# consilience-dev/llm-map-reduce-summarizer

Measured on AMD Instinct MI355X. Metric: chunks/sec (whole node) + end-to-end wall-clock, 10h transcript, Llama-3-8B, higher is better.
Workload: dtype bf16

## Files before the change

### llm_map_reduce_summarizer_amd/csrc/kernels/stream_gemm.hip

```cpp
#include "ar_common.h"

namespace {
enum { EPI_BF16 = 0, EPI_F32_PARTIAL = 1, EPI_SWIGLU = 2, EPI_SWIGLU_SPLIT = 3, EPI_RESID_SPLIT = 4 };
constexpr int SS_PARTS = 8;
constexpr int KBLK = 128;
constexpr int LDS_XTRA = 3 * 1024;
constexpr int LDS_BUDGET = 160 * 1024 - LDS_XTRA;

struct NormArgs {
    const float* ssq;
    int ssq_tiles;
    float inv_k, eps;
    bf16* resid;
    int ldr;
    float* ssp;
    int slab_m;
    mrsum_ar::TPPush tp;
};

template <int N>
__device__ __forceinline__ void wait_vmcnt() {
    static_assert(N >= 0 && N < 64, "vmcnt range");
    __builtin_amdgcn_s_waitcnt((N & 15) | (7 << 4) | (15 << 8) | ((N >> 4) << 14));
}
// ... 692 lines not shown
    f32x4 acc[MT];
#pragma unroll
    for (int m = 0; m < MT; ++m) acc[m] = f32x4{0.f, 0.f, 0.f, 0.f};

#pragma unroll
    for (int s = 0; s < D - 1; ++s) ISSUEP(s, min(s, nkb - 1));

    const uint32_t kb0 = (uint32_t)(ks / KBLK);
    uint32_t ex[P13_EXCAP], exkb = ~0u;
    if constexpr (BITS == 13) {
#pragma unroll
        for (int c = 0; c < P13_EXCAP; ++c) ex[c] = ~0u;
        if (nex > 0) {
#pragma unroll
            for (int c = 0; c < P13_EXCAP; ++c) {
                if (c < nex) ex[c] = __builtin_amdgcn_readfirstlane(exlist[ex0 + c]);
                const uint32_t kbc = ex[c] >> 18;
                if (kbc >= kb0) exkb = min(exkb, kbc);
            }
        }
    }

    const uint32_t base4 = (uint32_t)(base7 - 1) * 0x01010101u;
    const int r = lane & 15, g = lane >> 4;
    for (int j = 0; j < nkb; ++j) {
        if (j + D - 2 < nkb) wait_vmcnt<NI * (D - 2)>();
        else wait_vmcnt<0>();
        raw_barrier();
        if (j + D - 1 < nkb) ISSUEP((j + D - 1) % D, j + D - 1);
        const char* wl = lds + (j % D) * SLOT + w * TILE;
        const char* xl = lds + (j % D) * SLOT + WBYTES;
        const u32x4 lo0 = *reinterpret_cast<const u32x4*>(wl + 16 * lane);
        const u32x4 lo1 = *reinterpret_cast<const u32x4*>(wl + 1024 + 16 * lane);
        const u32x4 nb = *reinterpret_cast<const u32x4*>(wl + F::NIB + 16 * lane);
        u32x4 av[4];
        if constexpr (BITS == 14) {
            const u32x2 s2 = *reinterpret_cast<const u32x2*>(wl + F::TOP + 8 * lane);
            av[0] = p14_frag<0>(lo0[0], lo0[1], nb[0], s2.x, base4);
            av[1] = p14_frag<1>(lo0[2], lo0[3], nb[1], s2.x, base4);
            av[2] = p14_frag<0>(lo1[0], lo1[1], nb[2], s2.y, base4);
            av[3] = p14_frag<1>(lo1[2], lo1[3], nb[3], s2.y, base4);
        } else {
            const uint32_t sg = *reinterpret_cast<const uint32_t*>(wl + F::TOP + 4 * lane);
            av[0] = p13_frag<0>(lo0[0], lo0[1], nb[0], sg, base4);
            av[1] = p13_frag<1>(lo0[2], lo0[3], nb[1], sg, base4);
            av[2] = p13_frag<2>(lo1[0], lo1[1], nb[2], sg, base4);
            av[3] = p13_frag<3>(lo1[2], lo1[3], nb[3], sg, base4);
            if (kb0 + (uint32_t)j == exkb) {
                const uint32_t cur = exkb;
                exkb = ~0u;
#pragma unroll
                for (int c = 0; c < P13_EXCAP; ++c) {
                    uint32_t xc = ex[c];
                    asm volatile("" : "+s"(xc));
                    const uint32_t kbc = xc >> 18;
                    if (kbc == cur) {
                        const int sl = (xc >> 7) & 31;
                        const uint32_t v = lane == (int)((xc >> 12) & 63) ? (xc & 127u) << (8 + 16 * (sl & 1)) : 0u;
#pragma unroll
                        for (int i = 0; i < 4; ++i)
#pragma unroll
                            for (int d = 0; d < 4; ++d) av[i][d] |= sl >> 1 == 4 * i + d ? v : 0u;
                    } else if (kbc > cur) {
                        exkb = min(exkb, kbc);
                    }
                }
            }
        }
#pragma unroll
        for (int i = 0; i < 4; ++i) {
#pragma unroll
            for (int m = 0; m < MT; ++m) {
                const u32x4 bv = *reinterpret_cast<const u32x4*>(xl + img_off(16 * m + r, 4 * i + g));
                acc[m] = __builtin_amdgcn_mfma_f32_16x16x32_bf16(__builtin_bit_cast(bf16x8, av[i]),
                                                                 __builtin_bit_cast(bf16x8, bv), acc[m], 0, 0, 0);
            }
        }
    }
#undef ISSUEP

    stream_epilogue<MT, EPI, WPB>(acc, lds, s_ss, n0, M, out, ldo, parts, counters, e);
}

template <int BITS>
static int launch_packed(const void* x, int ldx, const void* W, int base7, const int* exoff, const uint32_t* exlist,
                         int N, int K, int M, void* out, int ldo, int epi, int splits, int wpb, void* parts,
                         int* counters, const float* ssq, int ssq_tiles, float eps, void* resid, int ldr, float* ssp,
                         void* ar, hipStream_t s) {
    if (M <= 0) return 0;
    if (wpb < 4 || wpb > 8 || M > 64 || K % KBLK || N % (16 * wpb) || splits < 1 || (K / KBLK) % splits ||
        epi < EPI_BF16 || epi > EPI_RESID_SPLIT || base7 < 1 || base7 > 128 - Packed<BITS>::WINDOW || ar)
        return (int)hipErrorInvalidValue;
    if (BITS == 13 && (!exoff || !exlist || K / KBLK >= 0x3fff)) return (int)hipErrorInvalidValue;
    const bool split_epi = epi == EPI_SWIGLU_SPLIT || epi == EPI_RESID_SPLIT;
    if (epi != EPI_F32_PARTIAL && !split_epi && splits != 1) return (int)hipErrorInvalidValue;
    if (split_epi && (!parts || !counters)) return (int)hipErrorInvalidValue;
    if (epi == EPI_RESID_SPLIT && (!resid || !ssp || ldr % 4)) return (int)hipErrorInvalidValue;
    if (ssq && (ssq_tiles <= 0 || ssq_tiles % (4 * SS_PARTS))) return (int)hipErrorInvalidValue;
    NormArgs e;
    e.ssq = ssq; e.ssq_tiles = ssq_tiles; e.inv_k = 1.f / (float)K; e.eps = eps;
    e.resid = (bf16*)resid; e.ldr = ldr; e.ssp = ssp; e.slab_m = 0;
    e.tp = mrsum_ar::tp_push_of(nullptr);
    const int kper = K / splits;
    const int mt = (M + 15) / 16;
    dim3 grid(N / (16 * wpb), splits), block(64 * wpb);
    auto X = (const bf16*)x;
    auto Wp = (const unsigned char*)W;
    auto P = (float*)parts;
#define L14(MT_, EPI_, WPB_)                                                                                      \
    stream_packed_kernel<BITS, MT_, EPI_, WPB_><<<grid, block, 0, s>>>(X, ldx, Wp, base7, exoff, exlist, K, M, out, \
                                                                       ldo, kper, P, counters, e)
#define BY_WPB14(MT_, EPI_)                         \
    switch (wpb) {                                  \
        case 4: L14(MT_, EPI_, 4); break;           \
        case 5: L14(MT_, EPI_, 5); break;           \
        case 6: L14(MT_, EPI_, 6); break;           \
        case 7: L14(MT_, EPI_, 7); break;           \
        default: L14(MT_, EPI_, 8); break;          \
    }
#define BY_EPI14(MT_)                                                      \
    if (epi == EPI_BF16) { BY_WPB14(MT_, EPI_BF16) }                       \
    else if (epi == EPI_F32_PARTIAL) { BY_WPB14(MT_, EPI_F32_PARTIAL) }    \
    else if (epi == EPI_SWIGLU) { BY_WPB14(MT_, EPI_SWIGLU) }              \
    else if (epi == EPI_SWIGLU_SPLIT) { BY_WPB14(MT_, EPI_SWIGLU_SPLIT) }  \
    else { BY_WPB14(MT_, EPI_RESID_SPLIT) }
    switch (mt) {
        case 1: BY_EPI14(1); break;
        case 2: BY_EPI14(2); break;
        case 3: BY_EPI14(3); break;
        default: BY_EPI14(4); break;
    }
#undef BY_EPI14
#undef BY_WPB14
#undef L14
    return (int)hipGetLastError();
}

MRSUM_API int mrsum_stream_p14(const void* x, int ldx, const void* W, int base7, int N, int K, int M, void* out,
                               int ldo, int epi, int splits, int wpb, void* parts, int* counters, const float* ssq,
                               int ssq_tiles, float eps, void* resid, int ldr, float* ssp, void* ar, hipStream_t s) {
    return launch_packed<14>(x, ldx, W, base7, nullptr, nullptr, N, K, M, out, ldo, epi, splits, wpb, parts, counters,
                             ssq, ssq_tiles, eps, resid, ldr, ssp, ar, s);
}

MRSUM_API int mrsum_stream_p13(const void* x, int ldx, const void* W, int base7, const int* exoff,
                               const unsigned int* exlist, int N, int K, int M, void* out, int ldo, int epi, int splits,
                               int wpb, void* parts, int* counters, const float* ssq, int ssq_tiles, float eps,
                               void* resid, int ldr, float* ssp, void* ar, hipStream_t s) {
    return launch_packed<13>(x, ldx, W, base7, exoff, exlist, N, K, M, out, ldo, epi, splits, wpb, parts, counters,
                             ssq, ssq_tiles, eps, resid, ldr, ssp, ar, s);
}

namespace {
__global__ __launch_bounds__(256) void p14_max_kernel(const uint4* __restrict__ W, size_t n16, int* __restrict__ stats) {
    uint32_t m = 0;
    for (size_t i = (size_t)blockIdx.x * blockDim.x + threadIdx.x; i < n16; i += (size_t)gridDim.x * blockDim.x) {
        const uint4 v = W[i];
        const uint32_t d[4] = {v.x, v.y, v.z, v.w};
#pragma unroll
        for (int c = 0; c < 4; ++c) m = max(m, max((d[c] >> 8) & 0x7fu, (d[c] >> 24) & 0x7fu));
    }
#pragma unroll
    for (int o = 32; o > 0; o >>= 1) m = max(m, (uint32_t)__shfl_xor((int)m, o, 64));
    if ((threadIdx.x & 63) == 0) atomicMax(stats, (int)m);
}

__global__ __launch_bounds__(64) void p14_pack_kernel(const bf16* __restrict__ W, int K, unsigned char* __restrict__ P,
                                                      int* __restrict__ stats) {
    const int lane = threadIdx.x, r = lane & 15, g = lane >> 4;
    const int nkb = K / KBLK;
    const size_t tile = blockIdx.x;
    const int G = (int)(tile / nkb), kb = (int)(tile % nkb);
    const int base7 = max(stats[0] - 30, 1);
    const uint4* src = reinterpret_cast<const uint4*>(W + (size_t)(16 * G + r) * K + (size_t)kb * KBLK + 8 * g);
    uint32_t lo[8], nb[4], s2[2] = {0u, 0u};
    int bad = 0;
#pragma unroll
    for (int i = 0; i < 4; ++i) {
        const uint4 v = src[4 * i];
        const uint32_t d[4] = {v.x, v.y, v.z, v.w};
        lo[2 * i] = lo[2 * i + 1] = nb[i] = 0u;
#pragma unroll
        for (int el = 0; el < 8; ++el) {
            const uint32_t wv = (d[el >> 1] >> (16 * (el & 1))) & 0xffffu;
            const int e7 = (wv >> 8) & 0x7f, c = e7 ? e7 - base7 + 1 : 0;
            bad += e7 && (c < 1 || c > 31);
            const uint32_t c5 = (uint32_t)c & 31u, sg = wv >> 15;
            const int b = el & 3, q = 2 * (i & 1) + (el >> 2);
            lo[2 * i + (el >> 2)] |= (wv & 0xffu) << (8 * b);
            nb[i] |= (c5 & 15u) << (8 * b + 4 * (el >> 2));
            s2[i >> 1] |= (c5 >> 4) << (8 * b + 4 - q) | sg << (8 * b + 7 - (q == 3 ? 7 : q));
        }
    }
    unsigned char* t = P + tile * P14_TILE;
    *reinterpret_cast<uint4*>(t + 16 * lane) = make_uint4(lo[0], lo[1], lo[2], lo[3]);
    *reinterpret_cast<uint4*>(t + 1024 + 16 * lane) = make_uint4(lo[4], lo[5], lo[6], lo[7]);
    *reinterpret_cast<uint4*>(t + P14_NIB + 16 * lane) = make_uint4(nb[0], nb[1], nb[2], nb[3]);
    *reinterpret_cast<uint2*>(t + P14_TWO + 8 * lane) = make_uint2(s2[0], s2[1]);
    if (bad) atomicAdd(stats + 1, bad);
}
}

MRSUM_API int mrsum_p14_pack(const void* W, int N, int K, void* packed, int* stats, hipStream_t s) {
    if (N <= 0 || K <= 0 || N % 16 || K % KBLK || !W || !packed || !stats) return (int)hipErrorInvalidValue;
    hipError_t rc = hipMemsetAsync(stats, 0, 2 * sizeof(int), s);
    if (rc != hipSuccess) return (int)rc;
    const size_t n16 = (size_t)N * K / 8;
    const int blocks = (int)((n16 + 255) / 256 < 4096 ? (n16 + 255) / 256 : 4096);
    p14_max_kernel<<<blocks, 256, 0, s>>>((const uint4*)W, n16, stats);
    p14_pack_kernel<<<(unsigned)((size_t)(N / 16) * (K / KBLK)), 64, 0, s>>>((const bf16*)W, K, (unsigned char*)packed,
                                                                              stats);
    return (int)hipGetLastError();
}

namespace {
__global__ __launch_bounds__(64) void p13_pack_kernel(const bf16* __restrict__ W, int K, unsigned char* __restrict__ P,
                                                      int* __restrict__ stats, int* __restrict__ excnt,
                                                      uint32_t* __restrict__ exbuf) {
    const int lane = threadIdx.x, r = lane & 15, g = lane >> 4;
    const int nkb = K / KBLK;
    const size_t tile = blockIdx.x;
    const int G = (int)(tile / nkb), kb = (int)(tile % nkb);
    const int base7 = max(stats[0] - 14, 1);
    const uint4* src = reinterpret_cast<const uint4*>(W + (size_t)(16 * G + r) * K + (size_t)kb * KBLK + 8 * g);
    uint32_t lo[8], nb[4], sg = 0u;
    int nexc = 0;
#pragma unroll
    for (int i = 0; i < 4; ++i) {
        const uint4 v = src[4 * i];
        const uint32_t d[4] = {v.x, v.y, v.z, v.w};
        lo[2 * i] = lo[2 * i + 1] = nb[i] = 0u;
#pragma unroll
        for (int el = 0; el < 8; ++el) {
// ... 41 lines not shown
```

### llm_map_reduce_summarizer_amd/ops/hip.py

```python

from __future__ import annotations

import ctypes
import os
from typing import Optional

import torch

from ._lib import kernels_lib
from .reference import Fp8Weight

_c_int, _c_float, _vp = ctypes.c_int, ctypes.c_float, ctypes.c_void_p

_SIGS = {
    "mrsum_rmsnorm": [_vp, _vp, _vp, _c_int, _c_int, _c_int, _c_int, _c_float, _vp],
    "mrsum_add_rmsnorm": [_vp, _vp, _vp, _vp, _c_int, _c_int, _c_int, _c_int, _c_float, _vp],
    "mrsum_rmsnorm_fp8": [_vp, _vp, _vp, _vp, _vp, _c_int, _c_int, _c_int, _c_int, _c_float, _c_int, _vp],
    "mrsum_rope_kv": [_vp, _c_int, _c_int, _vp, _vp, _vp, _c_int, _vp, _vp, _vp, _c_int, _c_int, _c_int, _c_int,
                      _c_int, _c_int, _vp],
    "mrsum_rope_kv_parts": [_vp, _c_int, _vp, _c_int, _c_int, _vp, _vp, _vp, _c_int, _vp, _vp, _vp, _c_int,
                            _c_int, _c_int, _c_int, _c_int, _vp],
    "mrsum_swiglu": [_vp, _vp, _c_int, _c_int, _vp],
    "mrsum_kv_scatter": [_vp, _c_int, _c_int, _c_int, _vp, _vp, _vp, _vp, _c_int, _vp],
    "mrsum_embed": [_vp, _vp, _vp, _c_int, _c_int, _c_int, _vp],
    "mrsum_attn_prefill": [_vp, _c_int, _vp, _vp, _c_int, _c_int, _vp, _c_int, _c_int, _c_int, _c_int, _c_float, _vp],
    "mrsum_attn_prefill_paged": [_vp, _c_int, _vp, _vp, _c_int, _c_int, _vp, _c_int, _c_int, _c_int, _c_int, _c_float,
                                 _vp,
                                 _vp, _vp, _c_int, _vp, _vp, _c_int, _vp],
    "mrsum_attn_decode_mfma": [_vp, _c_int, _vp, _vp, _vp, _c_int, _vp, _vp, _vp, _vp, _c_int, _c_int, _c_int,
                               _c_int, _c_int, _c_int, _c_int, _c_float, _vp, _c_int, _vp],
    "mrsum_attn_decode_rope": [_vp, _c_int, _vp, _vp, _vp, _vp, _c_int, _vp, _vp, _vp, _vp, _c_int, _c_int,
                               _c_int, _c_int, _c_int, _c_int, _c_int, _c_float, _vp, _c_int, _vp],
    "mrsum_skinny_gemm": [_vp, _c_int, _vp, _c_int, _c_int, _c_int, _vp, _c_int, _c_int, _c_int, _c_int, _vp, _c_int,
                          _c_float, _vp, _c_int, _vp, _vp, _c_int, _vp],
    "mrsum_skinny_resid_capacity_w": [_c_int],
    "mrsum_skinny_lds": [_vp, _c_int, _vp, _c_int, _c_int, _c_int, _vp, _c_int, _c_int, _c_int, _c_int, _vp],
    "mrsum_stream_gemm": [_vp, _c_int, _vp, _c_int, _c_int, _c_int, _vp, _c_int, _c_int, _c_int, _c_int, _vp, _vp,
                          _vp, _c_int, _c_float, _vp, _c_int, _vp, _c_int, _vp, _vp],
    "mrsum_stream_fp8": [_vp, _c_int, _vp, _vp, _c_int, _c_int, _c_int, _vp, _c_int, _c_int, _c_int, _c_int, _vp, _vp,
                         _vp, _c_int, _c_float, _vp, _c_int, _vp, _vp, _vp],
    "mrsum_stream_p14": [_vp, _c_int, _vp, _c_int, _c_int, _c_int, _c_int, _vp, _c_int, _c_int, _c_int, _c_int, _vp,
                         _vp, _vp, _c_int, _c_float, _vp, _c_int, _vp, _vp, _vp],
    "mrsum_p14_pack": [_vp, _c_int, _c_int, _vp, _vp, _vp],
    "mrsum_stream_p13": [_vp, _c_int, _vp, _c_int, _vp, _vp, _c_int, _c_int, _c_int, _vp, _c_int, _c_int, _c_int,
                         _c_int, _vp, _vp, _vp, _c_int, _c_float, _vp, _c_int, _vp, _vp, _vp],
    "mrsum_p13_pack": [_vp, _c_int, _c_int, _vp, _vp, _vp, _vp, _vp],
    "mrsum_skinny_fp8": [_vp, _c_int, _vp, _vp, _c_int, _c_int, _c_int, _vp, _c_int, _c_int, _c_int, _c_int, _vp,
                         _c_int, _c_float, _vp, _c_int, _vp, _vp, _c_int, _vp],
    "mrsum_skinny_fp8_resid_capacity": [],
    "mrsum_quant_fp8_rows": [_vp, _c_int, _vp, _vp, _c_int, _c_int, _vp],
    "mrsum_add_rmsnorm_parts": [_vp, _c_int, _vp, _vp, _vp, _c_int, _c_int, _c_int, _c_float, _vp],
    "mrsum_sample_keys": [_vp, _c_int, _c_int, _c_int, _c_int, _vp, _vp, _vp, _vp, _vp],
    "mrsum_sample_finish": [_vp, _vp, _vp, _vp, _vp, _vp, _c_int, _vp, _vp, _c_int, _vp],
    "mrsum_gemm": [_vp, _c_int, _vp, _c_int, _vp, _c_int, _c_int, _c_int, _c_int, _c_int, _c_int, _vp, _vp, _c_int,
                   _c_int, _vp],
    "mrsum_sample": [_vp, _c_int, _c_int, _c_int, _vp, _vp, _vp, _vp, _vp, _vp, _vp, _vp, _vp, _c_int, _vp, _vp,
                     _vp],
    "mrsum_penalize": [_vp, _c_int, _c_int, _c_int, _c_int, _vp, _c_int, _vp, _vp, _vp, _vp, _vp, _vp],
    "mrsum_penalize_scan": [_vp, _c_int, _c_int, _c_int, _c_int, _vp, _c_int, _vp, _vp, _vp, _vp, _vp, _vp],
    "mrsum_constrain": [_vp, _c_int, _c_int, _c_int, _c_int, _vp, _vp, _c_int, _vp, _vp, _vp, _vp, _vp, _vp, _vp],
    "mrsum_sample_finish_stops": [_vp, _vp, _vp, _vp, _vp, _vp, _c_int, _vp, _vp, _vp, _c_int, _vp],
    "mrsum_sample_keys_filtered": [_vp, _c_int, _c_int, _c_int, _vp, _vp, _vp, _vp, _vp, _vp, _vp, _vp, _vp, _vp],
    "mrsum_logprobs": [_vp, _c_int, _c_int, _c_int, _vp, _vp, _vp, _c_int, _vp, _vp, _vp, _vp, _vp, _vp, _vp, _vp],
    "mrsum_logprobs_pick": [_vp, _c_int, _c_int, _c_int, _vp, _c_int, _vp, _vp, _vp, _vp, _c_int, _vp],
    "mrsum_sample_thresh": [_vp, _c_int, _c_int, _c_int, _vp, _vp, _vp, _vp, _vp, _vp, _vp],
    "mrsum_sample_filtered": [_vp, _c_int, _c_int, _c_int, _vp, _vp, _vp, _vp, _vp, _vp, _vp, _vp, _vp, _vp, _vp,
                              _vp, _vp, _c_int, _vp, _vp, _vp],
}

_fns = {}


def _fn(name: str):
    f = _fns.get(name)
    if f is None:
        lib = kernels_lib()
        f = getattr(lib, name)
        f.argtypes = _SIGS[name]
        f.restype = ctypes.c_int
        _fns[name] = f
    return f


def _stream() -> int:
    return torch.cuda.current_stream().cuda_stream


def _p(t: Optional[torch.Tensor]) -> Optional[int]:
    return None if t is None else t.data_ptr()


DEBUG_SYNC = os.environ.get("MRSUM_DEBUG_SYNC", "0") == "1"


def _check(rc: int, name: str) -> None:
    if rc != 0:
        raise RuntimeError("%s launch failed: hipError %d" % (name, rc))
    if DEBUG_SYNC and not torch.cuda.is_current_stream_capturing():
        try:
            torch.cuda.synchronize()
        except RuntimeError as e:
            raise RuntimeError("%s: device error after the launch: %s" % (name, e)) from e


def _req(cond: bool, msg: str) -> None:
    if not cond:
        raise ValueError(msg)


def _bf16_cuda(*ts: torch.Tensor) -> None:
    for t in ts:
        _req(t.is_cuda and t.dtype == torch.bfloat16, "expected a bf16 CUDA tensor, got %s %s" % (t.dtype, t.device))


def _i32(*ts: torch.Tensor) -> None:
    for t in ts:
        _req(t.is_cuda and t.dtype == torch.int32 and t.is_contiguous(), "expected a contiguous int32 CUDA tensor")


def _rows_ok(x: torch.Tensor) -> None:
    _req(x.dim() == 2 and x.stride(1) == 1 and x.stride(0) % 8 == 0 and x.data_ptr() % 16 == 0,
         "expected a 2-D row-major tensor with 16-byte aligned rows")


def rmsnorm(x: torch.Tensor, w: torch.Tensor, eps: float, out: Optional[torch.Tensor] = None) -> torch.Tensor:
    _bf16_cuda(x, w)
    _rows_ok(x)
    T, D = x.shape
    _req(w.numel() == D and w.is_contiguous() and D % 8 == 0 and D <= 16384, "rmsnorm: bad weight / D")
    if out is None:
# ... 706 lines not shown
    return out


def _norm_args(x, norm):
    if norm is None:
        return None, 0, 0.0
    ssq, eps = norm
    _req(ssq.is_cuda and ssq.dtype == torch.float32 and ssq.is_contiguous() and ssq.dim() == 2
         and ssq.shape[0] == x.shape[0] and ssq.shape[1] % 32 == 0, "deferred norm: ssq must be fp32 [M, 32k]")
    return _p(ssq), ssq.shape[1], float(eps)


def _resid_args(x, N, epi, resid, ssp):
    if epi != EPI_RESID_SPLIT:
        return None, 0, None
    M = x.shape[0]
    _bf16_cuda(resid)
    _rows_ok(resid)
    _req(resid.shape == (M, N) and ssp is not None and ssp.dtype == torch.float32 and ssp.is_contiguous()
         and ssp.dim() == 2 and ssp.shape[0] == M, "resid split: residual [M, N] bf16 and ssp fp32 [M, tiles]")
    return _p(resid), resid.stride(0), _p(ssp)


def _stream_gemm(x, w, out, epi, splits, ldo, wpb, parts=None, counters=None, norm=None, resid=None, ssp=None,
                 ar=None):
    _bf16_cuda(x, w)
    _rows_ok(x)
    M, K = x.shape
    N = w.shape[0]
    if M > SKINNY_MAX_M and epi in (EPI_BF16, EPI_F32_PARTIAL, EPI_SWIGLU) and norm is None:
        ch = STREAM_TALL_M
        for r0 in range(0, M, ch):
            r1 = min(M, r0 + ch)
            if r1 - r0 > SKINNY_MAX_M:
                tw = tall_wpb(N, r1 - r0, splits)
                if tw is not None:
                    o = out[:, r0:r1] if epi == EPI_F32_PARTIAL else out[r0:r1]
                    _stream_launch(x[r0:r1], w, o, epi, splits, ldo, tw, None, None, None, None, None,
                                   M if epi == EPI_F32_PARTIAL else 0)
                    continue
            for c0 in range(r0, r1, SKINNY_MAX_M):
                c1 = min(r1, c0 + SKINNY_MAX_M)
                o = out[:, c0:c1] if epi == EPI_F32_PARTIAL else out[c0:c1]
                _stream_launch(x[c0:c1], w, o, epi, splits, ldo, wpb, None, None, None, None, None,
                               M if epi == EPI_F32_PARTIAL else 0)
        return out
    return _stream_launch(x, w, out, epi, splits, ldo, wpb, parts, counters, norm, resid, ssp, 0, ar)


STREAM_TALL_M = 128
_TALL_WPB = {6: (4, 5, 6), 8: (4, 5)}


def tall_wpb(N: int, M: int, splits: int) -> Optional[int]:
    mt = 6 if M <= 96 else 8
    best, key = None, None
    for wpb in _TALL_WPB[mt]:
        if N % (16 * wpb):
            continue
        grid = N // (16 * wpb) * splits
        k = (round(grid / (-(-grid // N_CU) * N_CU), 3), wpb)
        if key is None or k > key:
            best, key = wpb, k
    return best


def _stream_launch(x, w, out, epi, splits, ldo, wpb, parts, counters, norm, resid, ssp, slab_m, ar=None):
    M, K = x.shape
    N = w.shape[0]
    _req(w.is_contiguous() and w.shape[1] == K, "stream_gemm: weight must be [N, K] contiguous")
    tall_ok = M <= 128 and epi in (EPI_BF16, EPI_F32_PARTIAL, EPI_SWIGLU) and norm is None
    _req(1 <= M and (M <= SKINNY_MAX_M or tall_ok) and K % 128 == 0 and 4 <= wpb <= 8 and N % (16 * wpb) == 0
         and (K // 128) % splits == 0, "stream_gemm: unsupported shape M=%d N=%d K=%d S=%d wpb=%d"
         % (M, N, K, splits, wpb))
    if epi in (EPI_SWIGLU_SPLIT, EPI_RESID_SPLIT):
        _req(parts is not None and parts.shape == (splits, M, N) and parts.dtype == torch.float32
             and counters is not None and counters.numel() >= N // (16 * wpb), "stream_gemm: split-K scratch")
    if epi == EPI_RESID_SPLIT:
        _req(ssp.shape[1] == N // (16 * wpb), "stream_gemm: ssp tiles")
    sq, tiles, eps = _norm_args(x, norm)
    rp, ldr, sp = _resid_args(x, N, epi, resid, ssp)
    packed_ok = M <= SKINNY_MAX_M and not slab_m and ar is None
    p3 = p13_lookup(w) if _P13 else None
    if p3 is not None and packed_ok and p13_takes(p3.role, M):
        STATS["stream_p14"] += 1
        STATS["stream_p13"] += 1
        _check(_fn("mrsum_stream_p13")(_p(x), x.stride(0), _p(p3.packed), p3.base7, _p(p3.exoff), _p(p3.exlist), N, K,
                                       M, _p(out), ldo, epi, splits, wpb, _p(parts), _p(counters), sq, tiles, eps, rp,
                                       ldr, sp, None, _stream()), "stream_p13")
        return out
    pw = p14_lookup(w) if _P14 else None
    if pw is not None and packed_ok and p14_takes(pw.role, M):
        STATS["stream_p14"] += 1
        _check(_fn("mrsum_stream_p14")(_p(x), x.stride(0), _p(pw.packed), pw.base7, N, K, M, _p(out), ldo, epi, splits,
                                       wpb, _p(parts), _p(counters), sq, tiles, eps, rp, ldr, sp, None, _stream()),
               "stream_p14")
        return out
    STATS["stream_bf16"] += 1
    _check(_fn("mrsum_stream_gemm")(_p(x), x.stride(0), _p(w), N, K, M, _p(out), ldo, epi, splits, wpb, _p(parts),
                                    _p(counters), sq, tiles, eps, rp, ldr, sp, slab_m, ar, _stream()), "stream_gemm")
    return out


P14_ROLES = ("qkv", "o", "gate_up", "down", "lm_head")
_P14_PLAN = {("gate_up", 1), ("gate_up", 16), ("gate_up", 64), ("lm_head", 1), ("lm_head", 16),
             ("down", 1), ("down", 16)}
_P14 = {}


class PackedWeight:

    def __init__(self, w: torch.Tensor, packed: Optional[torch.Tensor], base7: int, packable: bool, role: str):
        self.w, self.packed, self.base7, self.packable, self.role = w, packed, base7, packable, role

    def nbytes(self) -> int:
        return self.packed.numel() if self.packed is not None else 0


def p14_enabled() -> bool:
    return os.environ.get("MRSUM_P14", P14_DEFAULT) == "1"


P14_DEFAULT = "1"


def p14_bucket(M: int) -> int:
    return 1 if M == 1 else 16 if M <= 16 else 64


def p14_role_used(role: str) -> bool:
    return any(r == role for r, _ in _P14_PLAN)


def p14_takes(role: str, M: int) -> bool:
    return p14_enabled() and (role, p14_bucket(M)) in _P14_PLAN


def p14_pack(w: torch.Tensor):
    _bf16_cuda(w)
    _req(w.dim() == 2 and w.is_contiguous() and w.shape[0] % 16 == 0 and w.shape[1] % 128 == 0,
         "p14_pack: expected a contiguous bf16 [16 n, 128 k] matrix")
    N, K = w.shape
    packed = torch.empty(N * K // 4 * 7, dtype=torch.uint8, device=w.device)
    stats = torch.zeros(2, dtype=torch.int32, device=w.device)
    _check(_fn("mrsum_p14_pack")(_p(w), N, K, _p(packed), _p(stats), _stream()), "p14_pack")
    mx, bad = (int(v) for v in stats.tolist())
    return packed, max(mx - 30, 1), bad


def p14_attach(w: torch.Tensor, role: str) -> PackedWeight:
    _req(role in P14_ROLES, "p14_attach: unknown role %r" % (role,))
    packed, base7, bad = p14_pack(w)
    if bad:
        print("p14: %s weight %s has %d elements outside the exponent window: bf16 kernel kept"
              % (role, tuple(w.shape), bad))
        return PackedWeight(w, None, base7, False, role)
    pw = _P14[(w.data_ptr(), w.shape[0], w.shape[1])] = PackedWeight(w, packed, base7, True, role)
    return pw


def p14_detach(w: torch.Tensor) -> None:
    _P14.pop((w.data_ptr(), w.shape[0], w.shape[1]), None)


def p14_lookup(w: torch.Tensor) -> Optional[PackedWeight]:
    return _P14.get((w.data_ptr(), w.shape[0], w.shape[1]))


_P13_PLAN = {("gate_up", 1), ("gate_up", 16), ("gate_up", 64), ("lm_head", 1), ("lm_head", 16),
             ("down", 1), ("down", 16)}
_P13 = {}
P13_EXCAP = 8
P13_DEFAULT = "1"


class Packed13Weight:

    def __init__(self, w, packed, base7, exoff, exlist, nex, packable, role):
        self.w, self.packed, self.base7, self.exoff, self.exlist = w, packed, base7, exoff, exlist
        self.nex, self.packable, self.role = nex, packable, role

    def nbytes(self) -> int:
        if self.packed is None:
            return 0
        return self.packed.numel() + 4 * (self.exoff.numel() + self.exlist.numel())


def p13_enabled() -> bool:
    return p14_enabled() and os.environ.get("MRSUM_P13", P13_DEFAULT) == "1"


def p13_role_used(role: str) -> bool:
    return any(r == role for r, _ in _P13_PLAN)


def p13_takes(role: str, M: int) -> bool:
    return p13_enabled() and (role, p14_bucket(M)) in _P13_PLAN


def p13_pack(w: torch.Tensor):
    _bf16_cuda(w)
    _req(w.dim() == 2 and w.is_contiguous() and w.shape[0] % 16 == 0 and w.shape[1] % 128 == 0
         and w.shape[1] // 128 < 0x3fff, "p13_pack: expected a contiguous bf16 [16 n, 128 k] matrix")
    N, K = w.shape
    G = N // 16
    packed = torch.empty(N * K // 8 * 13, dtype=torch.uint8, device=w.device)
    stats = torch.zeros(2, dtype=torch.int32, device=w.device)
    excnt = torch.zeros(G, dtype=torch.int32, device=w.device)
    exbuf = torch.full((G, P13_EXCAP), -1, dtype=torch.int32, device=w.device)
    _check(_fn("mrsum_p13_pack")(_p(w), N, K, _p(packed), _p(stats), _p(excnt), _p(exbuf), _stream()), "p13_pack")
    mx, nex = (int(v) for v in stats.tolist())
    exoff = torch.zeros(G + 1, dtype=torch.int32, device=w.device)
    exlist = torch.zeros(1, dtype=torch.int32, device=w.device)
    worst = 0
    if nex:
        worst = int(excnt.max())
        kept = excnt.clamp(max=P13_EXCAP)
        exoff[1:] = torch.cumsum(kept, 0)
        srt = torch.sort(exbuf.to(torch.int64) & 0xffffffff, dim=1).values
        keep = torch.arange(P13_EXCAP, device=w.device)[None, :] < kept[:, None]
        words = srt[keep]
        exlist = torch.where(words >= 2 ** 31, words - 2 ** 32, words).to(torch.int32).contiguous()
    return packed, max(mx - 14, 1), exoff, exlist, nex, worst


def p13_attach(w: torch.Tensor, role: str) -> Packed13Weight:
    _req(role in P14_ROLES, "p13_attach: unknown role %r" % (role,))
    packed, base7, exoff, exlist, nex, worst = p13_pack(w)
    if worst > P13_EXCAP:
        return Packed13Weight(w, None, base7, None, None, nex, False, role)
    pw = _P13[(w.data_ptr(), w.shape[0], w.shape[1])] = Packed13Weight(w, packed, base7, exoff, exlist, nex, True, role)
    return pw


def p13_detach(w: torch.Tensor) -> None:
    _P13.pop((w.data_ptr(), w.shape[0], w.shape[1]), None)


def packed_attach(w: torch.Tensor, role: str):
    if p13_enabled() and p13_role_used(role):
        p3 = p13_attach(w, role)
        if p3.packable:
            return p3
    return p14_attach(w, role) if p14_enabled() and p14_role_used(role) else None


def packed_detach(w: torch.Tensor) -> None:
    p13_detach(w)
    p14_detach(w)


def p13_lookup(w: torch.Tensor) -> Optional[Packed13Weight]:
    return _P13.get((w.data_ptr(), w.shape[0], w.shape[1]))


def linear_takes_norm(M: int, N: int, K: int) -> bool:
    return 1 <= M <= SKINNY_MAX_M and K % 128 == 0 and stream_config(N, K, splits=1) is not None


def linear(x: torch.Tensor, w: torch.Tensor, out: Optional[torch.Tensor] = None, norm=None) -> torch.Tensor:
    M, K = x.shape
    N = w.shape[0]
    _req(norm is None or linear_takes_norm(M, N, K), "linear: a deferred norm needs a stream-GEMM shape")
    tall = (SKINNY_MAX_M < M <= STREAM_TALL_M and K % 128 == 0 and norm is None
            and stream_config(N, K, splits=1) is not None and tall_wpb(N, M, 1) is not None)
    if (M > SKINNY_MAX_M and not tall) or M == 0 or K % 128:
        return gemm(x, w, out=out)
    if out is None:
        out = torch.empty(M, N, dtype=x.dtype, device=x.device)
    _req(out.is_contiguous() and out.shape == (M, N), "linear: bad out")
    if tall:
        return _stream_gemm(x, w, out, EPI_BF16, 1, N, tall_wpb(N, M, 1))
    cfg = stream_config(N, K, splits=1)
    if cfg is not None:
        return _stream_gemm(x, w, out, EPI_BF16, 1, N, cfg[0], norm=norm)
    nt = 2 if N % 32 == 0 and N >= 16384 else 1
    if N % (16 * nt):
        return gemm(x, w, out=out)
    return _skinny(x, w, out, EPI_BF16, nt, 1, N)


def linear_parts(x: torch.Tensor, w: torch.Tensor, splits: Optional[int] = None,
                 out: Optional[torch.Tensor] = None, nt: int = 1, kernel: str = "skinny", norm=None) -> torch.Tensor:
    M, K = x.shape
    N = w.shape[0]
    if splits is None:
        splits = choose_splits(N, K, nt if kernel == "skinny" else 4)
    if out is None:
        out = torch.empty(splits, M, N, dtype=torch.float32, device=x.device)
    _req(out.is_contiguous() and out.shape == (splits, M, N) and out.dtype == torch.float32, "linear_parts: bad out")
    if kernel == "stream":
        return _stream_gemm(x, w, out, EPI_F32_PARTIAL, splits, N, nt, norm=norm)
    _req(norm is None, "linear_parts: a deferred norm needs the stream kernel")
    if kernel == "lds":
        return _skinny_lds(x, w, out, EPI_F32_PARTIAL, splits, N)
    return _skinny(x, w, out, EPI_F32_PARTIAL, nt, splits, N)


_TILE_COUNTERS = {}


def _tile_counters(device, n: int) -> torch.Tensor:
    key = (str(device), n)
    t = _TILE_COUNTERS.get(key)
    if t is None:
        _req(not torch.cuda.is_current_stream_capturing(), "split-K SwiGLU tickets first used inside a capture")
        t = _TILE_COUNTERS[key] = torch.zeros(max(n, 1024), dtype=torch.int32, device=device)
    return t


def stream_swiglu_split(x: torch.Tensor, w_gu: torch.Tensor, out: torch.Tensor, wpb: int, splits: int,
                        norm=None) -> torch.Tensor:
    M, K = x.shape
    N = w_gu.shape[0]
    _req(out.is_contiguous() and out.shape == (M, N // 2), "stream_swiglu_split: bad out")
    parts = torch.empty(splits, M, N, dtype=torch.float32, device=x.device)
    cnt = _tile_counters(x.device, N // (16 * wpb))
    return _stream_gemm(x, w_gu, out, EPI_SWIGLU_SPLIT, splits, out.stride(0), wpb, parts=parts, counters=cnt,
                        norm=norm)


def stream_resid(x: torch.Tensor, w, residual: torch.Tensor, wpb: int, splits: int, tp=None) -> torch.Tensor:
    M = x.shape[0]
    fp8 = isinstance(w, Fp8Weight)
    N = (w.q if fp8 else w).shape[0]
    tiles = N // (16 * wpb)
    if tp is not None:
        STATS["tp_push"] += 1
    parts = torch.empty(splits, M, N, dtype=torch.float32, device=x.device)
    ssp = torch.empty(M, tiles, dtype=torch.float32, device=x.device)
    cnt = _tile_counters(x.device, tiles)
    if fp8:
        _stream_fp8(x, w, None, EPI_RESID_SPLIT, splits, 0, wpb, parts=parts, counters=cnt, resid=residual, ssp=ssp,
                    ar=tp)
    else:
        _stream_gemm(x, w, None, EPI_RESID_SPLIT, splits, 0, wpb, parts=parts, counters=cnt, resid=residual, ssp=ssp,
                     ar=tp)
    return ssp


_RESID_CAP = {}


def skinny_resid_capacity(N: Optional[int] = None) -> int:
    for waves in (4, 8):
        if waves not in _RESID_CAP:
            _RESID_CAP[waves] = int(_fn("mrsum_skinny_resid_capacity_w")(waves))
    return min(_RESID_CAP[4], _RESID_CAP[8])


def skinny_resid(x: torch.Tensor, w, residual: torch.Tensor, tp=None) -> torch.Tensor:
    N = w.shape[0]
    fp8 = isinstance(w, Fp8Weight)
    M = x.shape[0]
    ssp = torch.empty(M, N // 16, dtype=torch.float32, device=x.device)
    if tp is not None:
        cap = skinny_fp8_resid_capacity() if fp8 else skinny_resid_capacity(N)
        _req(N // 16 <= cap, "skinny_resid: TP-push grid of %d workgroups is not fully resident (capacity %d)"
             % (N // 16, cap))
        STATS["tp_push"] += 1
    if fp8:
        _skinny_fp8(x, w, None, EPI_SKINNY_RESID, 1, 1, 0, resid=residual, ssp=ssp, ar=tp)
    else:
        _skinny(x, w, None, EPI_SKINNY_RESID, 1, 1, 0, resid=residual, ssp=ssp, ar=tp)
    return ssp


def skinny_fp8_resid_capacity() -> int:
    if "fp8" not in _RESID_CAP:
        _RESID_CAP["fp8"] = int(_fn("mrsum_skinny_fp8_resid_capacity")())
    return _RESID_CAP["fp8"]


def linear_swiglu(x: torch.Tensor, w_gu: torch.Tensor, out: Optional[torch.Tensor] = None,
                  kernel: str = "skinny", wpb: int = 4, splits: int = 1, norm=None) -> torch.Tensor:
    M = x.shape[0]
    F2 = w_gu.shape[0]
    _req(norm is None or kernel in ("stream", "stream_split", "skinny"),
         "linear_swiglu: a deferred norm needs the stream or register-streaming kernel")
    if kernel == "gemm" or M > (STREAM_MAX_M_SWIGLU if kernel == "stream" else SKINNY_MAX_M):
        return gemm(x, w_gu, out=out, swiglu=True)
    if out is None:
        out = torch.empty(M, F2 // 2, dtype=x.dtype, device=x.device)
    _req(out.is_contiguous() and out.shape == (M, F2 // 2), "linear_swiglu: bad out")
    if kernel == "stream":
        return _stream_gemm(x, w_gu, out, EPI_SWIGLU, 1, F2 // 2, wpb, norm=norm)
    if kernel == "stream_split":
        return stream_swiglu_split(x, w_gu, out, wpb, splits, norm=norm)
    if kernel == "lds":
        return _skinny_lds(x, w_gu, out, EPI_SWIGLU, 1, F2 // 2)
    return _skinny(x, w_gu, out, EPI_SWIGLU, 1, 1, F2 // 2, norm=norm)


def add_rmsnorm_parts(parts: torch.Tensor, residual: torch.Tensor, w: torch.Tensor, eps: float,
                      out: Optional[torch.Tensor] = None) -> torch.Tensor:
    _req(parts.is_cuda and parts.dtype == torch.float32 and parts.is_contiguous() and parts.dim() == 3,
         "add_rmsnorm_parts: parts must be fp32 [S, T, D]")
    _bf16_cuda(residual, w)
    S, T, D = parts.shape
    _req(residual.shape == (T, D) and residual.is_contiguous() and w.numel() == D and w.is_contiguous()
         and D % 8 == 0 and D <= 16384, "add_rmsnorm_parts: shapes")
    if out is None:
        out = torch.empty(T, D, dtype=residual.dtype, device=residual.device)
    _bf16_cuda(out)
    _rows_ok(out)
    _req(out.shape == (T, D), "add_rmsnorm_parts: bad out shape")
    _check(_fn("mrsum_add_rmsnorm_parts")(_p(parts), S, _p(residual), _p(w), _p(out), T, D, out.stride(0), eps,
                                          _stream()), "add_rmsnorm_parts")
    return out


N_CU = 256
STATS = {"tp_push": 0, "stream_p14": 0, "stream_p13": 0, "stream_bf16": 0}


def stream_config(N: int, K: int, swiglu: bool = False, splits: Optional[int] = None, max_splits: int = 16):
    if K % 128:
        return None
    nkb = K // 128
    best, best_key = None, None
    for wpb in (4, 5, 6, 7, 8):
        if N % (16 * wpb):
            continue
        tiles = N // (16 * wpb)
        cands = [1] if swiglu else ([splits] if splits else range(1, max_splits + 1))
        for S in cands:
            if nkb % S:
                continue
            grid = tiles * S
            eff = grid / (-(-grid // N_CU) * N_CU)
            key = (round(eff, 3), -S, wpb if grid <= 2 * N_CU else -wpb)
            if best_key is None or key > best_key:
                best, best_key = (wpb, S), key
    if best is None or best_key[0] < 0.7:
        return None
    return best


def tp_resid_config(N: int, K: int):
    best, best_key = None, None
    for wpb in (4, 8):
        if N % (16 * wpb) or (N // (16 * wpb)) % 32:
            continue
        tiles = N // (16 * wpb)
        for S in range(1, 17):
            if (K // 128) % S:
                continue
            grid = tiles * S
            eff = grid / (-(-grid // N_CU) * N_CU)
            key = (round(eff, 3), -S, wpb)
            if best_key is None or key > best_key:
                best, best_key = (wpb, S), key
    return best


def swiglu_split_config(N: int, K: int):
    best, best_key = None, None
    for wpb in (4, 7, 8):
        if N % (16 * wpb):
            continue
        tiles = N // (16 * wpb)
        for S in (1, 2, 4, 8, 16):
            if (K // 128) % S or tiles * S > 2 * N_CU:
                continue
            grid = tiles * S
            key = (round(grid / (-(-grid // N_CU) * N_CU), 3), -S, wpb)
            if best_key is None or key > best_key:
                best, best_key = (wpb, S), key
    return best if best_key is not None and best_key[0] >= 0.7 else None


def plan(role: str, M: int, N: int, K: int, splits: Optional[int] = None, stream: bool = True):
    if M > (STREAM_MAX_M_SWIGLU if role == "gate_up" else STREAM_MAX_M) or K % 128:
        return ("gemm",)
    if role in ("o", "down") and M <= 16 and K <= 2048 and stream:
        s = splits or (2 if (K // 128) % 2 == 0 and K >= 1024 else 1)
        return ("skinny", 1, s)
    cfg = stream_config(N, K, swiglu=(role == "gate_up"), splits=splits) if stream else None
    if cfg is not None:
        return ("stream",) + cfg
    if M > SKINNY_MAX_M:
        return ("gemm",)
    if role == "gate_up" and stream and (K // 128) % 4 == 0:
        if N >= 7168 and N % 112 == 0 and (M > 8 or N // 112 * 4 <= N_CU):
            return ("stream_split", 7, 4)
        if N % 64 == 0 and M > 16:
            return ("stream_split", 4, 4)
    blocks = K // 128

    def div(s):
        while blocks % s:
            s -= 1
        return s

    if role == "qkv":
        if M <= 8:
# ... 187 lines not shown
```

Baseline: 2.272.

## Add producer-warp activation ring to packed stream GEMM for mid-size batches

Measured after the change: 2.286, median of 6. About the same (+0.6%).

```diff
diff --git a/llm_map_reduce_summarizer_amd/csrc/kernels/stream_gemm.hip b/llm_map_reduce_summarizer_amd/csrc/kernels/stream_gemm.hip
--- a/llm_map_reduce_summarizer_amd/csrc/kernels/stream_gemm.hip
+++ b/llm_map_reduce_summarizer_amd/csrc/kernels/stream_gemm.hip
@@ -798,7 +798,186 @@
     stream_epilogue<MT, EPI, WPB>(acc, lds, s_ss, n0, M, out, ldo, parts, counters, e);
 }
 
-template <int BITS>
+namespace {
+constexpr int xring_dw(int tile, int mt, int wpb) {
+    const int d = (LDS_BUDGET - 3 * mt * 4096) / (wpb * tile);
+    return d < 8 ? d : 8;
+}
+constexpr int xring_dx(int tile, int mt, int wpb) {
+    const int d = (LDS_BUDGET - xring_dw(tile, mt, wpb) * wpb * tile) / (mt * 4096);
+    return d < 4 ? d : 4;
+}
+
+template <int EPI>
+__device__ __forceinline__ void xring_loader_epilogue(const NormArgs& e, const char* lds) {
+    if (e.ssq) __syncthreads();
+    if constexpr (EPI == EPI_SWIGLU_SPLIT || EPI == EPI_RESID_SPLIT) {
+        __syncthreads();
+        __syncthreads();
+        if constexpr (EPI == EPI_RESID_SPLIT) {
+            if (*reinterpret_cast<const int*>(lds) != 0) __syncthreads();
+        }
+    }
+}
+}
+
+template <int BITS, int MT, int EPI, int WPB, bool PROBE = false>
+__global__ __launch_bounds__(64 * (WPB + 1), 1) void stream_packed_xring_kernel(
+    const bf16* __restrict__ x, int ldx, const unsigned char* __restrict__ W, int base7, const int* __restrict__ exoff,
+    const uint32_t* __restrict__ exlist, int K, int M, void* __restrict__ out, int ldo, int kper,
+    float* __restrict__ parts, int* __restrict__ counters, const NormArgs e) {
+    using F = Packed<BITS>;
+    static_assert(MT >= 2 && MT <= 4, "one row tile: stream_packed_kernel");
+    constexpr int TILE = F::TILE;
+    constexpr int R = 16 * WPB, BM = 16 * MT;
+    constexpr int WBYTES = WPB * TILE, XBYTES = BM * 256;
+    constexpr int DW = xring_dw(TILE, MT, WPB), DX = xring_dx(TILE, MT, WPB);
+    static_assert(DW >= 3 && DW <= 8 && DX >= 2 && DX <= 4, "ring depths");
+    constexpr int XOFF = DW * WBYTES;
+    static_assert(XOFF + DX * XBYTES <= LDS_BUDGET, "LDS budget");
+    constexpr int XP = 2 * BM / 8;
+    constexpr int NI = F::NW;
+    static_assert(NI * (DW - 2) < 64 && XP * (DX - 2) < 64, "vmcnt range");
+    __shared__ __attribute__((aligned(1024))) char lds[XOFF + DX * XBYTES + LDS_XTRA];
+    float* const s_ss = reinterpret_cast<float*>(lds + XOFF + DX * XBYTES + 1024);
+
+    const int tid = threadIdx.x, lane = tid & 63;
+    const int w = __builtin_amdgcn_readfirstlane(tid >> 6);
+    const int n0 = blockIdx.x * R;
+    const int ks = blockIdx.y * kper;
+    const int nkb = kper / KBLK;
+
+    if (w == WPB) {
+        const int prow = lane >> 3, pslot = lane & 7;
+        const bf16* xsrc[XP];
+#pragma unroll
+        for (int q = 0; q < XP; ++q) {
+            const int row = 8 * (q >> 1) + prow;
+            xsrc[q] = x + (size_t)min(row, M - 1) * ldx + ks + 8 * (8 * (q & 1) + (pslot ^ prow));
+        }
+#define ISSUEX(slot, kb)                                                                             \
+    {                                                                                                \
+        char* base = lds + XOFF + (slot) * XBYTES;                                                   \
+        _Pragma("unroll") for (int q = 0; q < XP; ++q) glds16(xsrc[q] + (kb) * KBLK, base + q * 1024); \
+    }
+#pragma unroll
+        for (int s = 0; s < DX - 1; ++s) ISSUEX(s, min(s, nkb - 1));
+        for (int j = 0; j < nkb; ++j) {
+            if (j + DX - 2 < nkb) wait_vmcnt<XP * (DX - 2)>();
+            else wait_vmcnt<0>();
+            raw_barrier();
+            if constexpr (!PROBE) {
+                if (j + DX - 1 < nkb) ISSUEX((j + DX - 1) % DX, j + DX - 1);
+            }
+        }
+#undef ISSUEX
+        xring_loader_epilogue<EPI>(e, lds);
+        return;
+    }
+
+    int ex0 = 0, nex = 0;
+    if constexpr (BITS == 13) {
+        const int G = n0 / 16 + w;
+        ex0 = exoff[G];
+        nex = exoff[G + 1] - ex0;
+    }
+
+    const unsigned char* const wsrc = W + ((size_t)(n0 / 16 + w) * (K / KBLK) + ks / KBLK) * TILE;
+#define ISSUEW(slot, kb)                                                                             \
+    {                                                                                                \
+        char* wb = lds + (slot) * WBYTES + w * TILE;                                                 \
+        const unsigned char* ws = wsrc + (size_t)(kb) * TILE;                                        \
+        glds16<2>(ws + 16 * lane, wb);                                                               \
+        glds16<2>(ws + 1024 + 16 * lane, wb + 1024);                                                 \
+        glds16<2>(ws + F::NIB + 16 * lane, wb + F::NIB);                                             \
+        glds4<2>(ws + F::TOP + 4 * lane, wb + F::TOP);                                               \
+        if constexpr (BITS == 14) glds4<2>(ws + F::TOP + 256 + 4 * lane, wb + F::TOP + 256);         \
+    }
+
+    f32x4 acc[MT];
+#pragma unroll
+    for (int m = 0; m < MT; ++m) acc[m] = f32x4{0.f, 0.f, 0.f, 0.f};
+
+#pragma unroll
+    for (int s = 0; s < DW - 1; ++s) ISSUEW(s, min(s, nkb - 1));
+
+    const uint32_t kb0 = (uint32_t)(ks / KBLK);
+    uint32_t ex[P13_EXCAP], exkb = ~0u;
+    if constexpr (BITS == 13) {
+#pragma unroll
+        for (int c = 0; c < P13_EXCAP; ++c) ex[c] = ~0u;
+        if (nex > 0) {
+#pragma unroll
+            for (int c = 0; c < P13_EXCAP; ++c) {
+                if (c < nex) ex[c] = __builtin_amdgcn_readfirstlane(exlist[ex0 + c]);
+                const uint32_t kbc = ex[c] >> 18;
+                if (kbc >= kb0) exkb = min(exkb, kbc);
+            }
+        }
+    }
+
+    const uint32_t base4 = (uint32_t)(base7 - 1) * 0x01010101u;
+    const int r = lane & 15, g = lane >> 4;
+    for (int j = 0; j < nkb; ++j) {
+        if (j + DW - 2 < nkb) wait_vmcnt<NI * (DW - 2)>();
+        else wait_vmcnt<0>();
+        raw_barrier();
+        if (j + DW - 1 < nkb) ISSUEW((j + DW - 1) % DW, j + DW - 1);
+        const char* wl = lds + (j % DW) * WBYTES + w * TILE;
+        const char* xl = lds + XOFF + (j % DX) * XBYTES;
+        const u32x4 lo0 = *reinterpret_cast<const u32x4*>(wl + 16 * lane);
+        const u32x4 lo1 = *reinterpret_cast<const u32x4*>(wl + 1024 + 16 * lane);
+        const u32x4 nb = *reinterpret_cast<const u32x4*>(wl + F::NIB + 16 * lane);
+        u32x4 av[4];
+        if constexpr (BITS == 14) {
+            const u32x2 s2 = *reinterpret_cast<const u32x2*>(wl + F::TOP + 8 * lane);
+            av[0] = p14_frag<0>(lo0[0], lo0[1], nb[0], s2.x, base4);
+            av[1] = p14_frag<1>(lo0[2], lo0[3], nb[1], s2.x, base4);
+            av[2] = p14_frag<0>(lo1[0], lo1[1], nb[2], s2.y, base4);
+            av[3] = p14_frag<1>(lo1[2], lo1[3], nb[3], s2.y, base4);
+        } else {
+            const uint32_t sg = *reinterpret_cast<const uint32_t*>(wl + F::TOP + 4 * lane);
+            av[0] = p13_frag<0>(lo0[0], lo0[1], nb[0], sg, base4);
+            av[1] = p13_frag<1>(lo0[2], lo0[3], nb[1], sg, base4);
+            av[2] = p13_frag<2>(lo1[0], lo1[1], nb[2], sg, base4);
+            av[3] = p13_frag<3>(lo1[2], lo1[3], nb[3], sg, base4);
+            if (kb0 + (uint32_t)j == exkb) {
+                const uint32_t cur = exkb;
+                exkb = ~0u;
+#pragma unroll
+                for (int c = 0; c < P13_EXCAP; ++c) {
+                    uint32_t xc = ex[c];
+                    asm volatile("" : "+s"(xc));
+                    const uint32_t kbc = xc >> 18;
+                    if (kbc == cur) {
+                        const int sl = (xc >> 7) & 31;
+                        const uint32_t v = lane == (int)((xc >> 12) & 63) ? (xc & 127u) << (8 + 16 * (sl & 1)) : 0u;
+#pragma unroll
+                        for (int i = 0; i < 4; ++i)
+#pragma unroll
+                            for (int d = 0; d < 4; ++d) av[i][d] |= sl >> 1 == 4 * i + d ? v : 0u;
+                    } else if (kbc > cur) {
+                        exkb = min(exkb, kbc);
+                    }
+                }
+            }
+        }
+#pragma unroll
+        for (int i = 0; i < 4; ++i) {
+#pragma unroll
+            for (int m = 0; m < MT; ++m) {
+                const u32x4 bv = *reinterpret_cast<const u32x4*>(xl + img_off(16 * m + r, 4 * i + g));
+                acc[m] = __builtin_amdgcn_mfma_f32_16x16x32_bf16(__builtin_bit_cast(bf16x8, av[i]),
+                                                                 __builtin_bit_cast(bf16x8, bv), acc[m], 0, 0, 0);
+            }
+        }
+    }
+#undef ISSUEW
+
+    stream_epilogue<MT, EPI, WPB>(acc, lds, s_ss, n0, M, out, ldo, parts, counters, e);
+}
+
+template <int BITS, bool XR = false>
 static int launch_packed(const void* x, int ldx, const void* W, int base7, const int* exoff, const uint32_t* exlist,
                          int N, int K, int M, void* out, int ldo, int epi, int splits, int wpb, void* parts,
                          int* counters, const float* ssq, int ssq_tiles, float eps, void* resid, int ldr, float* ssp,
@@ -808,6 +987,7 @@
         epi < EPI_BF16 || epi > EPI_RESID_SPLIT || base7 < 1 || base7 > 128 - Packed<BITS>::WINDOW || ar)
         return (int)hipErrorInvalidValue;
     if (BITS == 13 && (!exoff || !exlist || K / KBLK >= 0x3fff)) return (int)hipErrorInvalidValue;
+    if (XR && M <= 16) return (int)hipErrorInvalidValue;
     const bool split_epi = epi == EPI_SWIGLU_SPLIT || epi == EPI_RESID_SPLIT;
     if (epi != EPI_F32_PARTIAL && !split_epi && splits != 1) return (int)hipErrorInvalidValue;
     if (split_epi && (!parts || !counters)) return (int)hipErrorInvalidValue;
@@ -819,13 +999,18 @@
     e.tp = mrsum_ar::tp_push_of(nullptr);
     const int kper = K / splits;
     const int mt = (M + 15) / 16;
-    dim3 grid(N / (16 * wpb), splits), block(64 * wpb);
+    dim3 grid(N / (16 * wpb), splits), block(64 * (wpb + (XR ? 1 : 0)));
     auto X = (const bf16*)x;
     auto Wp = (const unsigned char*)W;
     auto P = (float*)parts;
-#define L14(MT_, EPI_, WPB_)                                                                                      \
-    stream_packed_kernel<BITS, MT_, EPI_, WPB_><<<grid, block, 0, s>>>(X, ldx, Wp, base7, exoff, exlist, K, M, out, \
-                                                                       ldo, kper, P, counters, e)
+#define L14(MT_, EPI_, WPB_)                                                                                          \
+    if constexpr (XR) {                                                                                               \
+        if constexpr ((MT_) >= 2)                                                                                     \
+            stream_packed_xring_kernel<BITS, MT_, EPI_, WPB_><<<grid, block, 0, s>>>(X, ldx, Wp, base7, exoff, exlist, \
+                                                                                     K, M, out, ldo, kper, P, counters, e); \
+    } else                                                                                                            \
+        stream_packed_kernel<BITS, MT_, EPI_, WPB_><<<grid, block, 0, s>>>(X, ldx, Wp, base7, exoff, exlist, K, M, out, \
+                                                                           ldo, kper, P, counters, e)
 #define BY_WPB14(MT_, EPI_)                         \
     switch (wpb) {                                  \
         case 4: L14(MT_, EPI_, 4); break;           \
@@ -865,6 +1050,54 @@
                                void* resid, int ldr, float* ssp, void* ar, hipStream_t s) {
     return launch_packed<13>(x, ldx, W, base7, exoff, exlist, N, K, M, out, ldo, epi, splits, wpb, parts, counters,
                              ssq, ssq_tiles, eps, resid, ldr, ssp, ar, s);
+}
+
+MRSUM_API int mrsum_stream_p14_xring(const void* x, int ldx, const void* W, int base7, int N, int K, int M, void* out,
+                                     int ldo, int epi, int splits, int wpb, void* parts, int* counters,
+                                     const float* ssq, int ssq_tiles, float eps, void* resid, int ldr, float* ssp,
+                                     void* ar, hipStream_t s) {
+    return launch_packed<14, true>(x, ldx, W, base7, nullptr, nullptr, N, K, M, out, ldo, epi, splits, wpb, parts,
+                                   counters, ssq, ssq_tiles, eps, resid, ldr, ssp, ar, s);
+}
+
+MRSUM_API int mrsum_stream_p13_xring(const void* x, int ldx, const void* W, int base7, const int* exoff,
+                                     const unsigned int* exlist, int N, int K, int M, void* out, int ldo, int epi,
+                                     int splits, int wpb, void* parts, int* counters, const float* ssq, int ssq_tiles,
+                                     float eps, void* resid, int ldr, float* ssp, void* ar, hipStream_t s) {
+    return launch_packed<13, true>(x, ldx, W, base7, exoff, exlist, N, K, M, out, ldo, epi, splits, wpb, parts,
+                                   counters, ssq, ssq_tiles, eps, resid, ldr, ssp, ar, s);
+}
+
+MRSUM_API int mrsum_xring_depths(int bits, int mt, int wpb, int* dw, int* dx) {
+    if ((bits != 13 && bits != 14) || mt < 2 || mt > 4 || wpb < 4 || wpb > 8 || !dw || !dx)
+        return (int)hipErrorInvalidValue;
+    const int tile = bits == 13 ? P13_TILE : P14_TILE;
+    *dw = xring_dw(tile, mt, wpb);
+    *dx = xring_dx(tile, mt, wpb);
+    return 0;
+}
+
+MRSUM_API int mrsum_stream_p13_xring_probe(const void* x, int ldx, const void* W, int base7, const int* exoff,
+                                           const unsigned int* exlist, int N, int K, int M, void* out, int ldo, int wpb,
+                                           hipStream_t s) {
+    if (M <= 32 || M > 48 || K % KBLK || (wpb != 4 && wpb != 7 && wpb != 8) || N % (16 * wpb) || base7 < 1 ||
+        base7 > 128 - Packed<13>::WINDOW || !exoff || !exlist || K / KBLK >= 0x3fff)
+        return (int)hipErrorInvalidValue;
+    NormArgs e;
+    e.ssq = nullptr; e.ssq_tiles = 0; e.inv_k = 1.f / (float)K; e.eps = 0.f;
+    e.resid = nullptr; e.ldr = 0; e.ssp = nullptr; e.slab_m = 0;
+    e.tp = mrsum_ar::tp_push_of(nullptr);
+    dim3 grid(N / (16 * wpb)), block(64 * (wpb + 1));
+#define LP(WPB_)                                                                                        \
+    stream_packed_xring_kernel<13, 3, EPI_BF16, WPB_, true><<<grid, block, 0, s>>>(                     \
+        (const bf16*)x, ldx, (const unsigned char*)W, base7, exoff, exlist, K, M, out, ldo, K, nullptr, nullptr, e)
+    switch (wpb) {
+        case 4: LP(4); break;
+        case 7: LP(7); break;
+        default: LP(8); break;
+    }
+#undef LP
+    return (int)hipGetLastError();
 }
 
 namespace {
diff --git a/llm_map_reduce_summarizer_amd/ops/hip.py b/llm_map_reduce_summarizer_amd/ops/hip.py
--- a/llm_map_reduce_summarizer_amd/ops/hip.py
+++ b/llm_map_reduce_summarizer_amd/ops/hip.py
@@ -45,7 +45,14 @@
     "mrsum_stream_p13": [_vp, _c_int, _vp, _c_int, _vp, _vp, _c_int, _c_int, _c_int, _vp, _c_int, _c_int, _c_int,
                          _c_int, _vp, _vp, _vp, _c_int, _c_float, _vp, _c_int, _vp, _vp, _vp],
     "mrsum_p13_pack": [_vp, _c_int, _c_int, _vp, _vp, _vp, _vp, _vp],
-    "mrsum_skinny_fp8": [_vp, _c_int, _vp, _vp, _c_int, _c_int, _c_int, _vp, _c_int, _c_int, _c_int, _c_int, _vp,
+    "mrsum_stream_p14_xring": [_vp, _c_int, _vp, _c_int, _c_int, _c_int, _c_int, _vp, _c_int, _c_int, _c_int, _c_int,
+                               _vp, _vp, _vp, _c_int, _c_float, _vp, _c_int, _vp, _vp, _vp],
+    "mrsum_stream_p13_xring": [_vp, _c_int, _vp, _c_int, _vp, _vp, _c_int, _c_int, _c_int, _vp, _c_int, _c_int, _c_int,
+                               _c_int, _vp, _vp, _vp, _c_int, _c_float, _vp, _c_int, _vp, _vp, _vp],
+    "mrsum_xring_depths": [_c_int, _c_int, _c_int, _vp, _vp],
+    "mrsum_stream_p13_xring_probe": [_vp, _c_int, _vp, _c_int, _vp, _vp, _c_int, _c_int, _c_int, _vp, _c_int, _c_int,
+                                     _vp],
+    "mrsum_skinny_fp8":[_vp, _c_int, _vp, _vp, _c_int, _c_int, _c_int, _vp, _c_int, _c_int, _c_int, _c_int, _vp,
                          _c_int, _c_float, _vp, _c_int, _vp, _vp, _c_int, _vp],
     "mrsum_skinny_fp8_resid_capacity": [],
     "mrsum_quant_fp8_rows": [_vp, _c_int, _vp, _vp, _c_int, _c_int, _vp],
@@ -918,16 +925,33 @@
     rp, ldr, sp = _resid_args(x, N, epi, resid, ssp)
     packed_ok = M <= SKINNY_MAX_M and not slab_m and ar is None
     p3 = p13_lookup(w) if _P13 else None
-    if p3 is not None and packed_ok and p13_takes(p3.role, M):
+    xr = p3 is not None and packed_ok and p13_enabled() and xring_takes(p3.role, M)
+    if p3 is not None and packed_ok and (xr or p13_takes(p3.role, M)):
         STATS["stream_p14"] += 1
         STATS["stream_p13"] += 1
+        if xr:
+            STATS["stream_xring"] += 1
+            wx = _XRING_WPB.get(p3.role, wpb) if epi == EPI_BF16 and splits == 1 else wpb
+            wx = wx if N % (16 * wx) == 0 else wpb
+            _check(_fn("mrsum_stream_p13_xring")(_p(x), x.stride(0), _p(p3.packed), p3.base7, _p(p3.exoff),
+                                                 _p(p3.exlist), N, K, M, _p(out), ldo, epi, splits, wx, _p(parts),
+                                                 _p(counters), sq, tiles, eps, rp, ldr, sp, None, _stream()),
+                   "stream_p13_xring")
+            return out
         _check(_fn("mrsum_stream_p13")(_p(x), x.stride(0), _p(p3.packed), p3.base7, _p(p3.exoff), _p(p3.exlist), N, K,
                                        M, _p(out), ldo, epi, splits, wpb, _p(parts), _p(counters), sq, tiles, eps, rp,
                                        ldr, sp, None, _stream()), "stream_p13")
         return out
     pw = p14_lookup(w) if _P14 else None
-    if pw is not None and packed_ok and p14_takes(pw.role, M):
+    xr = pw is not None and packed_ok and p14_enabled() and xring_takes(pw.role, M)
+    if pw is not None and packed_ok and (xr or p14_takes(pw.role, M)):
         STATS["stream_p14"] += 1
+        if xr:
+            STATS["stream_xring"] += 1
+            _check(_fn("mrsum_stream_p14_xring")(_p(x), x.stride(0), _p(pw.packed), pw.base7, N, K, M, _p(out), ldo,
+                                                 epi, splits, wpb, _p(parts), _p(counters), sq, tiles, eps, rp, ldr,
+                                                 sp, None, _stream()), "stream_p14_xring")
+            return out
         _check(_fn("mrsum_stream_p14")(_p(x), x.stride(0), _p(pw.packed), pw.base7, N, K, M, _p(out), ldo, epi, splits,
                                        wpb, _p(parts), _p(counters), sq, tiles, eps, rp, ldr, sp, None, _stream()),
                "stream_p14")
@@ -1090,6 +1114,29 @@
     return _P13.get((w.data_ptr(), w.shape[0], w.shape[1]))
 
 
+_XRING_PLAN = {("gate_up", 64), ("lm_head", 64)}
+_XRING_WPB = {"lm_head": 8}
+XRING_DEFAULT = "1"
+XRING_LDS_BUDGET = 160 * 1024 - 3 * 1024
+_XRING_TILE = {13: 3328, 14: 3584}
+_XRING_NW = {13: 4, 14: 5}
+
+
+def xring_depths(bits: int, mt: int, wpb: int):
+    wslot, xslot = wpb * _XRING_TILE[bits], mt * 4096
+    dw = min(8, (XRING_LDS_BUDGET - 3 * xslot) // wslot)
+    dx = min(4, (XRING_LDS_BUDGET - dw * wslot) // xslot)
+    return dw, dx
+
+
+def xring_enabled() -> bool:
+    return os.environ.get("MRSUM_XRING", XRING_DEFAULT) == "1"
+
+
+def xring_takes(role: str, M: int) -> bool:
+    return 16 < M <= SKINNY_MAX_M and xring_enabled() and (role, p14_bucket(M)) in _XRING_PLAN
+
+
 def linear_takes_norm(M: int, N: int, K: int) -> bool:
     return 1 <= M <= SKINNY_MAX_M and K % 128 == 0 and stream_config(N, K, splits=1) is not None
 
@@ -1247,7 +1294,7 @@
 
 
 N_CU = 256
-STATS = {"tp_push": 0, "stream_p14": 0, "stream_p13": 0, "stream_bf16": 0}
+STATS = {"tp_push": 0, "stream_p14": 0, "stream_p13": 0, "stream_bf16": 0, "stream_xring": 0}
 
 
 def stream_config(N: int, K: int, swiglu: bool = False, splits: Optional[int] = None, max_splits: int = 16):
```
